# Cyan4973/FiniteStateEntropy

Measured on AMD Instinct MI355X. Metric: MB/s encode+decode per GPU on 32KB probagen blocks; bit-exact vs CPU ref, higher is better.
Workload: dtype u8; 1 GPU; probagen Proba14, 100000 x 32KB blocks per GPU, FSE encode+decode (one-shot calls at the reference's default limits: tableLog 11, decode maxLog 12), bit-exact check; blocks_per_gpu=100000, block_bytes=32768, codec=fse, parity=fse: roundtrip-all-blocks

## Files before the change

### finitestateentropy_amd/csrc/bitreader.h

```cpp
#pragma once
#include "dev_common.h"

enum { BR_UNFINISHED = 0, BR_END_OF_BUFFER = 1, BR_COMPLETED = 2, BR_OVERFLOW = 3 };

DEV u64 ldg64u(const u8* p) { u64 v; __builtin_memcpy(&v, p, 8); return v; }

struct BitReader {
    const u8* base; size_t size; size_t at; u64 win; u32 used;
    DEV size_t init(const u8* src, size_t n)
    {
        base = src; size = n; at = 0; win = 0; used = 0;
        if (n < 1) return FERR(srcSize_wrong);
        const u32 last = src[n - 1];
        if (n >= 8) {
            at = n - 8; win = ldg64u(src + at);
            if (last == 0) return FERR(GENERIC);
            used = 8 - hibit32(last);
        } else {
            for (size_t k = 0; k < n; ++k) win |= (u64)src[k] << (8 * k);
            if (last == 0) return FERR(corruption_detected);
            used = 8 - hibit32(last) + (u32)(8 - n) * 8;
        }
        return n;
    }
    DEV u32 read(u32 nb)
    {
        const u32 v = (u32)((win >> ((64u - used - nb) & 63u)) & (((u64)1 << nb) - 1));
        used += nb; return v;
    }
    DEV u32 read_fast(u32 nb)
    {
        const u32 v = (u32)((win << (used & 63u)) >> ((64u - nb) & 63u));
        used += nb; return v;
    }
    DEV int reload()
    {
        if (used > 64) return BR_OVERFLOW;
        if (at >= 8) { at -= used >> 3; used &= 7; win = ldg64u(base + at); return BR_UNFINISHED; }
        if (at == 0) return used < 64 ? BR_END_OF_BUFFER : BR_COMPLETED;
        u32 nbytes = used >> 3; int res = BR_UNFINISHED;
        if (at < nbytes) { nbytes = (u32)at; res = BR_END_OF_BUFFER; }
        at -= nbytes; used -= nbytes * 8; win = ldg64u(base + at);
        return res;
    }
};

DEV u32 fse_step(u32& state, BitReader& r, const u32* cells, bool fast)
{
    const u32 c = cells[state];
    const u32 nb = c >> 24;
    const u32 low = fast ? r.read_fast(nb) : r.read(nb);
    state = (c & 0xFFFFu) + low;
    return (c >> 16) & 0xFFu;
}
```

### finitestateentropy_amd/csrc/fse_decode.hip

```cpp
#include "internal.h"
#include <atomic>

#include "bitreader.h"

#ifndef FSE_SYM_L1
#define FSE_SYM_L1 1
#endif
#ifndef FSE_DEC_RING
#define FSE_DEC_RING 64
#endif
#define FSE_IN_RING 256
#define FSE_IN_RING_LOG 8
#define FSE_IN_CHUNK 64
#define FSE_IN_LANES (FSE_IN_CHUNK / 4)
#define FSE_IN_MIRROR 16
#ifndef FSE_CHECK_EVERY
#define FSE_CHECK_EVERY 16
#endif
#ifndef FSE_PHASE_UNROLL
#define FSE_PHASE_UNROLL 16
#endif
#define FSE_FINISH_EVERY 2
#ifndef FSE_DEC_LDS_KB
#define FSE_DEC_LDS_KB 160
// ... 133 lines not shown
DEV int ctl_peek(const int* p) { const int v = __hip_atomic_load(p, __ATOMIC_RELAXED, __HIP_MEMORY_SCOPE_WORKGROUP); __asm__ volatile("" ::: "memory"); return v; }
DEV void ctl_store(u32* p, u32 v) { __hip_atomic_store(p, v, __ATOMIC_RELEASE, __HIP_MEMORY_SCOPE_WORKGROUP); }
DEV u64 ctl_load2(const u32* p) { return __hip_atomic_load((const u64*)p, __ATOMIC_ACQUIRE, __HIP_MEMORY_SCOPE_WORKGROUP); }
DEV u64 ctl_peek2(const u32* p) { const u64 v = __hip_atomic_load((const u64*)p, __ATOMIC_RELAXED, __HIP_MEMORY_SCOPE_WORKGROUP); __asm__ volatile("" ::: "memory"); return v; }
DEV void ctl_store2(u32* p, u32 lo, u32 hi) { __hip_atomic_store((u64*)p, (u64)lo | ((u64)hi << 32), __ATOMIC_RELEASE, __HIP_MEMORY_SCOPE_WORKGROUP); }
DEV void ctl_store(int* p, int v) { __hip_atomic_store(p, v, __ATOMIC_RELEASE, __HIP_MEMORY_SCOPE_WORKGROUP); }

#define FSE_SRV_G 4
#ifndef FSE_FLUSH_MIN
#define FSE_FLUSH_MIN 32u
#endif
static_assert(FSE_SRV_WAVES * FSE_SRV_G == FSE_MAXG, "every block of a workgroup has a service wave");
static_assert((FSE_DEC_RING & (FSE_DEC_RING - 1)) == 0 && FSE_DEC_RING % FSE_CHECK_EVERY == 0, "ring positions wrap by masking; a phase never wraps");
DEV void fse_ring_put(u32* rg, int off, u32 w)
{
    const u32 j = (u32)off & (FSE_IN_RING - 1);
    rg[j >> 2] = w;
    if (j < FSE_IN_MIRROR) rg[(FSE_IN_RING + j) >> 2] = w;
}
DEV void fse_ring_put_rev(u32* rg, int Sg, int off, u32 w) { fse_ring_put(rg, ((Sg + 3) & ~3) - 4 - off, __brev(w)); }
DEV u32 fse_scratch_slot_claim(const FseDecArgs& a, u32* flagsSh)
{
    u32 slot = (u32)blockIdx.x % a.nSlots;
    for (;;) {
        const u32 bit = 1u << (slot & 31u);
        const u32 old = __hip_atomic_fetch_or(a.slotBitmap + (slot >> 5), bit, __ATOMIC_ACQUIRE, __HIP_MEMORY_SCOPE_AGENT);
        if (!(old & bit)) break;
        slot = slot + 1 == a.nSlots ? 0 : slot + 1;
    }
    flagsSh[6] = slot;
#if FSE_SYM_L1
    __builtin_amdgcn_fence(__ATOMIC_ACQUIRE, "agent");
#endif
    return slot;
}
DEV void fse_scratch_slot_done(const FseDecArgs& a, u32* flagsSh, int lane)
{
    if (lane == 0 && atomicAdd(&flagsSh[7], 1u) == FSE_SRV_WAVES + FSE_DEC_WAVES - 1) {
        const u32 slot = flagsSh[6];
        __hip_atomic_fetch_and(a.slotBitmap + (slot >> 5), ~(1u << (slot & 31u)), __ATOMIC_RELEASE, __HIP_MEMORY_SCOPE_AGENT);
    }
}
DEV u32 srv_rl(u32 v, int l) { return (u32)__builtin_amdgcn_readlane((int)v, l); }
DEV unsigned long long srv_rl64(unsigned long long v, int l) { return (unsigned long long)srv_rl((u32)v, l) | ((unsigned long long)srv_rl((u32)(v >> 32), l) << 32); }
template <bool TIMED, bool CALLER>
DEV void fse_decode_service(const FseDecArgs& a, u8* ldsb, DecCtl* ctlAll, u32 slotBytes, u32 ringOff, u32 inOff, int lane, int g0, bool rev, u32* flagsSh)
{
    const int myG = g0 + (lane < FSE_SRV_G ? lane : 0);
    DecCtl* const ctl = ctlAll + (myG < a.G ? myG : 0);
    const unsigned long long inBits = ((unsigned long long)ctl->inHi << 32) | ctl->inLo;
    const unsigned long long outBits = ((unsigned long long)ctl->outHi << 32) | ctl->outLo;
    const unsigned long long tabBits = ((unsigned long long)ctl->symHi << 32) | ctl->symLo;
    const int S32 = ctl->S32;
    int validLo = ctl->initValidLo;
    u32 flushed = 0, fpos = 0;
    bool live = lane < FSE_SRV_G && myG < a.G && !(ctl->pubPofs >> 31);

    static_assert(64 / FSE_IN_LANES == FSE_SRV_G, "one 16-lane group per block of a service wave");
    const int grp = lane / FSE_IN_LANES, sub = lane % FSE_IN_LANES;
    const int SgK = __shfl(S32, grp, WAVE);
    const gbl_u8_ptr igK = (gbl_u8_ptr)(uintptr_t)__shfl(inBits, grp, WAVE);
    u32* const rgK = (u32*)(ldsb + (size_t)(g0 + grp) * slotBytes + inOff);
    {   const bool liveK = (__ballot(live) >> grp) & 1ull;
        const int vlo = __shfl(validLo, grp, WAVE);
#pragma unroll
        for (int c = 0; c < FSE_IN_RING / FSE_IN_CHUNK; ++c) {
            const int off = liveK ? vlo + FSE_IN_CHUNK * c + 4 * sub : -1;
            if (off >= 0 && off + 4 <= SgK) { const u32 w = gbl_load_u32(igK + off); if (rev) fse_ring_put_rev(rgK, SgK, off, w); else fse_ring_put(rgK, off, w); }
            else if (off >= 0 && off < SgK) {
                u32 w = 0;
                for (int i = 0; i < 3; ++i) if (off + i < SgK) w |= (u32)igK[off + i] << (8 * i);
                if (rev) fse_ring_put_rev(rgK, SgK, off, w); else fse_ring_put(rgK, off, w);
            }
        }
        if (live) ctl_store(&ctl->srvValidLo, validLo);
    }

    int nextOff = __shfl(validLo, grp, WAVE) - FSE_IN_CHUNK + 4 * sub;
    u32 pend = 0;
    if (((__ballot(live) >> grp) & 1ull) && nextOff >= 0 && nextOff + 4 <= SgK) pend = gbl_load_u32(igK + nextOff);
    u32 yq[FSE_SRV_G][4];
#pragma unroll
    for (int l = 0; l < FSE_SRV_G; ++l) { yq[l][0] = yq[l][1] = yq[l][2] = yq[l][3] = 0; }
    unsigned long long sBusy = 0, sIdle = 0, nBusy = 0, sA = 0;
    (void)sBusy; (void)sIdle; (void)nBusy; (void)sA;
    TIMING(sA = __builtin_readcyclecounter(););
    for (;;) {
        u32 pp = 0x80000000u, it = flushed;
        if (live) { const u64 pub = ctl_load2(&ctl->pubIters); it = (u32)pub; pp = (u32)(pub >> 32); }
        const bool fin = (pp >> 31) != 0;
        const int P = (int)(pp & 0x7FFFFFFFu);
        const u32 avail = it - flushed;
        const bool wantFlush = live && (avail >= FSE_FLUSH_MIN || (fin && avail > 0));
        const bool wantFill = live && !fin && validLo > 0 && P + 4 <= validLo + (FSE_IN_RING - FSE_IN_CHUNK);
        const unsigned long long fm = __ballot(wantFlush), rm = __ballot(wantFill);
        if (live && fin && avail == 0) live = false;
        if (!(fm | rm)) {
            if (!__any(live)) break;
            __builtin_amdgcn_s_sleep(4);
            TIMING(const unsigned long long sB = __builtin_readcyclecounter(); sIdle += sB - sA; sA = sB;);
            continue;
        }
        const bool fillK = (rm >> grp) & 1ull;
        if (rm) {
            if (fillK) { if (rev) fse_ring_put_rev(rgK, SgK, nextOff, pend); else fse_ring_put(rgK, nextOff, pend); }
            if (wantFill) { validLo -= FSE_IN_CHUNK; ctl_store(&ctl->srvValidLo, validLo); }
            if (fillK) {
                nextOff -= FSE_IN_CHUNK;
                pend = 0;
                if (nextOff >= 0 && nextOff + 4 <= SgK) pend = gbl_load_u32(igK + nextOff);
            }
        }
#pragma unroll
        for (int l = 0; l < FSE_SRV_G; ++l) {
            if (!((fm >> l) & 1ull)) continue;
            const u32 cnt = srv_rl(avail, l), fp_g = srv_rl(fpos, l);
            const gbl_u8_ptr tg = (gbl_u8_ptr)(uintptr_t)srv_rl64(tabBits, l);
            if ((u32)lane < cnt) {
                u32 ri = fp_g + (u32)lane;
                ri = ri >= FSE_DEC_RING ? ri - FSE_DEC_RING : ri;
                const u32* const rw = (const u32*)(ldsb + (size_t)(g0 + l) * slotBytes + ringOff) + 4u * (ri >> 1) + (ri & 1u);
                uint2 rec; rec.x = rw[0]; rec.y = rw[2];
                const u32 x0 = __builtin_amdgcn_ubfe(rec.x, 1u, a.ldsLog), x1 = __builtin_amdgcn_ubfe(rec.x, 17u, a.ldsLog);
                const u32 x2 = __builtin_amdgcn_ubfe(rec.y, 1u, a.ldsLog), x3 = __builtin_amdgcn_ubfe(rec.y, 17u, a.ldsLog);
#if FSE_SYM_L1
                yq[l][0] = tg[x0]; yq[l][2] = tg[x1]; yq[l][1] = tg[x2]; yq[l][3] = tg[x3];
#else
                if (CALLER) {
                    yq[l][0] = __hip_atomic_load(tg + x0, __ATOMIC_RELAXED, __HIP_MEMORY_SCOPE_AGENT); yq[l][2] = __hip_atomic_load(tg + x1, __ATOMIC_RELAXED, __HIP_MEMORY_SCOPE_AGENT);
                    yq[l][1] = __hip_atomic_load(tg + x2, __ATOMIC_RELAXED, __HIP_MEMORY_SCOPE_AGENT); yq[l][3] = __hip_atomic_load(tg + x3, __ATOMIC_RELAXED, __HIP_MEMORY_SCOPE_AGENT);
                } else { yq[l][0] = tg[x0]; yq[l][2] = tg[x1]; yq[l][1] = tg[x2]; yq[l][3] = tg[x3]; }
#endif
            }
        }
        if (wantFlush) { ctl_store(&ctl->srvFlushed, it); }
#pragma unroll
        for (int l = 0; l < FSE_SRV_G; ++l) {
            if (!((fm >> l) & 1ull)) continue;
            const u32 cnt = srv_rl(avail, l), fl_g = srv_rl(flushed, l);
            gbl_u8_w_ptr const og = (gbl_u8_w_ptr)(uintptr_t)(srv_rl64(outBits, l) + 4ull * fl_g);
            if ((u32)lane < cnt) {
                const u32 w = yq[l][0] | (yq[l][1] << 8) | (yq[l][2] << 16) | (yq[l][3] << 24);
                gbl_store_u32(og + 4u * lane, w);
            }
        }
        if (wantFlush) { fpos += it - flushed; fpos = fpos >= FSE_DEC_RING ? fpos - FSE_DEC_RING : fpos; flushed = it; }
        TIMING(const unsigned long long sB = __builtin_readcyclecounter(); sBusy += sB - sA; sA = sB; ++nBusy;);
    }
    TIMING(if (lane == 0 && g0 == 0) { atomicAdd(&g_decTiming[5], sBusy); atomicAdd(&g_decTiming[6], sIdle); });
    if (CALLER) fse_scratch_slot_done(a, flagsSh, lane);
}

struct FseCellsRef { const u32* cells;
    DEV void get(u32 st, u32& ns, u32& nb, u32& sym) const { const u32 c = cells[st]; ns = c & 0xFFFFu; sym = (c >> 16) & 0xFFu; nb = c >> 24; } };
struct FseCellsCompact { const u16* A; const u8* syms;
    DEV void get(u32 st, u32& ns, u32& nb, u32& sym) const { const u32 c = A[st]; ns = c & 0xFFFu; nb = c >> 12; sym = syms[st]; } };
struct FseCellsRev { const u16* A; const u8* syms; u32 tl, cellShift;
    DEV void get(u32 st, u32& ns, u32& nb, u32& sym) const { const u32 i = __brev(st) >> (32u - tl); const u32 c = A[i]; nb = c & 31u; ns = __brev(c >> cellShift) >> (32u - tl); sym = syms[i]; } };
template <class Cells>
DEV u32 fse_tail_step(const Cells& t, u32& state, BitReader& r, bool fast)
{
    u32 ns, nb, sym;
    t.get(state, ns, nb, sym);
    const u32 low = fast ? r.read_fast(nb) : r.read(nb);
    state = ns + low;
    return sym;
}
template <class Cells>
DEV size_t fse_tail(const Cells& t, u32 s1, u32 s2, BitReader& r, u8* out, long op, long omax, bool fast)
{
    for (;;) {
        const int st = r.reload();
        if (!((st == BR_UNFINISHED) & (op < omax - 3))) break;
        u32 w = fse_tail_step(t, s1, r, fast);
        w |= fse_tail_step(t, s2, r, fast) << 8;
        w |= fse_tail_step(t, s1, r, fast) << 16;
        w |= fse_tail_step(t, s2, r, fast) << 24;
        __builtin_memcpy(out + op, &w, 4);
        op += 4;
    }
    for (;;) {
        if (op > omax - 2) return FERR(dstSize_tooSmall);
        out[op++] = (u8)fse_tail_step(t, s1, r, fast);
        if (r.reload() == BR_OVERFLOW) { out[op++] = (u8)fse_tail_step(t, s2, r, fast); return (size_t)op; }
        if (op > omax - 2) return FERR(dstSize_tooSmall);
        out[op++] = (u8)fse_tail_step(t, s2, r, fast);
        if (r.reload() == BR_OVERFLOW) { out[op++] = (u8)fse_tail_step(t, s1, r, fast); return (size_t)op; }
    }
}

template <bool FAST, bool TIMED, bool CALLER, bool VIEW = false>
__global__ __launch_bounds__(FSE_DEC_THREADS) void k_fse_decode(FseDecArgs a)
{
    extern __shared__ __attribute__((aligned(16))) u32 lds[];
    const int tid = threadIdx.x, lane = tid & 63, wave = tid >> 6;
    unsigned long long tBorn = 0, wBorn = 0;
    (void)tBorn; (void)wBorn;
    TIMING(tBorn = __builtin_readcyclecounter(); wBorn = wall_clock64(););
    const size_t first = (size_t)blockIdx.x * a.G;
    static_assert(FSE_DBINS % 4 == 0, "the bin lengths are read as 16-byte vectors");
    size_t nTot = a.nBlocks, q0 = first;
    u32 bin0 = 0, cnt0 = 0xFFFFFFFFu;
    if (a.count) {
        uint4 cv[FSE_DBINS / 4];
#pragma unroll
        for (u32 i = 0; i < FSE_DBINS / 4; ++i) cv[i] = ((const uint4*)a.count)[i];
        u64 before = 0;
        bool found = false;
#pragma unroll
        for (u32 i = 0; i < FSE_DBINS; ++i) {
            const uint4 v = cv[i >> 2];
            const u32 c = (i & 3u) == 0 ? v.x : (i & 3u) == 1 ? v.y : (i & 3u) == 2 ? v.z : v.w;
            const bool here = !found & (((u64)first < before + c) | (i == FSE_DBINS - 1));
            bin0 = here ? i : bin0; q0 = here ? (size_t)((u64)first - before) : q0; cnt0 = here ? c : cnt0;
            found |= here;
            before += c;
        }
        nTot = (size_t)before;
    }
    if (first >= nTot) return;
    auto slotBlock = [&](size_t g) -> size_t {
        if (!a.list) return first + g;
        size_t q = q0 + g; u32 i = bin0;
        if (q >= cnt0) {
            while (i < FSE_DBINS - 1) { const u32 c = a.count[i]; if (q < c) break; q -= c; ++i; }
        }
        return a.list[(size_t)i * a.nBlocks + q];
    };
    u8* const lds8 = (u8*)lds;
    const u32 tabStride = 2u << a.ldsLog;
    DecCtl* const ctlAll = (DecCtl*)(lds8 + (size_t)a.G * tabStride);
    u8* const ldsb = (u8*)ctlAll + (size_t)a.G * sizeof(DecCtl);
    const u32 slotBytes = a.slotU32 * 4u;
    const u32 ringOff = 0;
    const u32 inOff = FSE_DEC_RING * 8;

    u32* const flagsSh = (u32*)(ldsb + (size_t)a.G * slotBytes);
    if (tid < 6 || tid == 7) flagsSh[tid] = 0;
    const bool decWave = wave < FSE_DEC_WAVES;
    u8* const tlSh = (u8*)(flagsSh + 8);
    if (CALLER) {
        __syncthreads();
        bool mine = false;
        if (tid >= 64 && tid < 64 + a.G) {
            const size_t g = (size_t)tid - 64;
            u32 tl = 0xFFu;
            if (first + g < nTot) {
                const size_t bi = slotBlock(g);
                if (!(a.onlyDeclined && a.results[bi] != FSE_DECLINED)) {
                    const u32 t0 = a.dtables[bi * a.dtStrideU32] & 0xFFFFu;
                    if (t0 <= a.ldsLog && t0 >= a.tlMin) tl = t0;
                    else if (t0 > a.maxTableLog && a.tlMin == 0 && !a.onlyDeclined) a.results[bi] = FERR(tableLog_tooLarge);
                }
            }
            tlSh[g] = (u8)tl;
            mine = tl != 0xFFu;
        }
        if (mine) flagsSh[1] = 1u;
        u32 slot = 0;
        if (tid == 0) slot = fse_scratch_slot_claim(a, flagsSh);
        __syncthreads();
        if (!flagsSh[1]) {
            if (tid == 0) __hip_atomic_fetch_and(a.slotBitmap + (slot >> 5), ~(1u << (slot & 31u)), __ATOMIC_RELEASE, __HIP_MEMORY_SCOPE_AGENT);
            return;
        }
    }
    else __syncthreads();
    u8* const symSlot = CALLER ? a.symScratch + (size_t)flagsSh[6] * a.scratchSlotBytes : nullptr;
    {   u64 badBits = 0, declBits = 0; bool anyNb0 = false;
        if (!CALLER) {
            const size_t nTab = nTot - first < (size_t)a.G ? nTot - first : (size_t)a.G;
            if (tabStride >= 1024u) {
                const u32 ppt = tabStride >> 10;
                const u32 nPieces = (u32)nTab * ppt;
                for (u32 p = (u32)wave; p < nPieces; p += FSE_DEC_THREADS / 64) {
                    const u32 g = p / ppt, k = p - g * ppt;
                    const size_t bi = slotBlock(g);
                    const u8* const src = (const u8*)(a.atab + (bi << a.maxTableLog)) + 1024u * k + 16u * (u32)lane;
                    __builtin_amdgcn_global_load_lds((const __attribute__((address_space(1))) void*)src,
                                                     (__attribute__((address_space(3))) void*)(lds8 + 1024u * p), 16, 0, 0);
                }
            }
            else {
            uint4* const dstv = (uint4*)lds8;
            const u32 vptLog = a.ldsLog - 3u;
            const u32 nvec = (u32)nTab << vptLog;
            constexpr u32 MAXV = (FSE_MAXG * 512u / 16u + FSE_DEC_THREADS - 1) / FSE_DEC_THREADS;
            uint4 buf[MAXV];
#pragma unroll
            for (u32 k = 0; k < MAXV; ++k) {
                const u32 idx = tid + k * FSE_DEC_THREADS;
                if (idx < nvec) {
                    const size_t sl = first + (idx >> vptLog);
                    const size_t bi = slotBlock(sl - first);
                    buf[k] = ((const uint4*)(a.atab + (bi << a.maxTableLog)))[idx & ((1u << vptLog) - 1u)];
                }
            }
#pragma unroll
            for (u32 k = 0; k < MAXV; ++k) { const u32 idx = tid + k * FSE_DEC_THREADS; if (idx < nvec) dstv[idx] = buf[k]; }
            }
            if (!FAST) for (size_t g = 0; g < nTab; ++g) {
                const u32 st = a.meta[slotBlock(g)].state; anyNb0 |= st != 0 && !(st & 2u); }
        }
        else {
            const size_t nTab = nTot - first < (size_t)a.G ? nTot - first : (size_t)a.G;
            constexpr u32 QL = 2048u / 4u / 64u;
            if (!decWave) for (u32 g = (u32)wave - FSE_DEC_WAVES; g < (u32)nTab; g += FSE_SRV_WAVES) {
                const u32 tl = tlSh[g];
                if (tl == 0xFFu) continue;
                const u32 ts = 1u << tl;
                const u32* const t = a.dtables + slotBlock(g) * a.dtStrideU32;
                u8* const slotB = lds8 + (size_t)g * tabStride;
                u16* const A = (u16*)slotB;
                u8* const symOut = symSlot + ((size_t)g << a.ldsLog);
                bool bad = false, nbz = false;
                if (FAST && tl >= 4u) {
                    const u32 sR = 32u - tl;
                    const u32 qo[4] = { 0u, 1u << (tl - 1u), 1u << (tl - 2u), 3u << (tl - 2u) };
                    const u32 passes = ts > 2048u ? ts / 2048u : 1u;
                    u32 acc = 0, minNb = 15u;
                    uint4 cv[QL];
                    for (u32 h = 0; h < passes; ++h) {
#pragma unroll
                        for (u32 j = 0; j < QL; ++j) {
                            const u32 i0 = 2048u * h + 4u * ((u32)lane + 64u * j);
                            cv[j] = make_uint4(0, 0, 0, 0);
                            if (i0 < ts) __builtin_memcpy(&cv[j], t + 1 + i0, 16);
                        }
#pragma unroll
                        for (u32 j = 0; j < QL; ++j) {
                            const u32 i0 = 2048u * h + 4u * ((u32)lane + 64u * j);
                            if (i0 >= ts) continue;
                            const u32 r0 = __brev(i0) >> sR;
                            const u32 cw[4] = { cv[j].x, cv[j].y, cv[j].z, cv[j].w };
#pragma unroll
                            for (u32 q = 0; q < 4; ++q) {
                                const u32 c = cw[q], ns = c & 0xFFFFu, nb = c >> 24;
                                acc |= (ns >> tl) | ((tl - nb) >> 5) | (ns & ((1u << (nb & 31u)) - 1u));
                                minNb = nb < minNb ? nb : minNb;
                                slotB[r0 | qo[q]] = (u8)(c >> 16);
                            }
// ... 80 lines not shown
            s1 = r.read(tl); r.reload();
            s2 = r.read(tl); r.reload();
        }
    }

    __builtin_amdgcn_s_waitcnt(0x0f70);
    __syncthreads();
    const u64 badMask = (u64)flagsSh[2] | ((u64)flagsSh[3] << 32);
    const u64 declMask = (u64)flagsSh[4] | ((u64)flagsSh[5] << 32);
    const bool nb0 = flagsSh[0] != 0;
    if (CALLER && owner && a.declineNb0 && ((declMask >> gsl) & 1ull)) { if (half == 0) a.results[b] = FSE_DECLINED; owner = false; }

    const bool bulkOk = owner && S < (1ull << 28) && !((badMask >> gsl) & 1ull) && !(FAST && !compact && ((declMask >> gsl) & 1ull));
    const int Bstart = bulkOk ? (int)(8u * ((u32)r.at + 8u)) - (int)r.used : 0;
    const long groups0 = (omax - 3 - op + 3) / 4;
    bool can = bulkOk && (FAST ? Bstart >= 65 + 48 * (FSE_CHECK_EVERY - 1) : r.at >= 24 + 6 * FSE_CHECK_EVERY + 8) && groups0 >= FSE_CHECK_EVERY;
    bool can2 = FAST && bulkOk && Bstart >= 65 + 48 * (FSE_FINISH_EVERY - 1) && groups0 >= FSE_FINISH_EVERY;
    const bool everBulk = can || can2;
    BulkState bs; bs.q = 0; bs.bq = 0;
    {   const u32 st = half ? s2 : s1;
        bs.s = tabOff + 2u * (FAST ? __brev(st) >> (32u - (tl ? tl : 1u)) : st); }
    const u32 inA = (u32)((uintptr_t)in & 3u);
    const u32 R8 = 8u * (((u32)S + inA + 3u) & ~3u);
    u32 P = 0;
    long groups = 0;
    u32 iters = 0;
    int validLo = 0;
    if (everBulk) {
        const u32 B = 8u * ((u32)r.at + 8u + inA) - r.used;
        bs.q = 4u * (B >> 5) - 8u; bs.bq = B & 31u; P = R8 - B;
        groups = (omax - 3 - op + 3) >> 2;
        const int c0 = (int)((0 - ((uintptr_t)in - inA)) & (FSE_IN_CHUNK - 1));
        validLo = (((int)bs.q + 8 - 112 - c0) & ~(FSE_IN_CHUNK - 1)) + c0;
    }
    DecCtl* const ctl = ctlAll + (gsl < a.G ? gsl : 0);
    if (decWave && (lane >> 1) < ppw && gsl < a.G && half == 0) {
        ctl->pubIters = 0; ctl->pubPofs = everBulk ? bs.q + 8u : 0x80000000u;
        ctl->srvFlushed = 0; ctl->srvValidLo = 0x7FFFFFFF;
        ctl->initValidLo = validLo; ctl->S32 = (int)(S < (1ull << 31) ? S + inA : 0);
        const unsigned long long ib = (unsigned long long)(uintptr_t)(in - inA), ob = (unsigned long long)(uintptr_t)out, tb = (unsigned long long)(uintptr_t)syms;
        ctl->inLo = (u32)ib; ctl->inHi = (u32)(ib >> 32); ctl->outLo = (u32)ob; ctl->outHi = (u32)(ob >> 32); ctl->symLo = (u32)tb; ctl->symHi = (u32)(tb >> 32);
    }
    __syncthreads();
    if (!decWave) { fse_decode_service<TIMED, CALLER>(a, ldsb, ctlAll, slotBytes, ringOff, inOff, lane, (wave - FSE_DEC_WAVES) * FSE_SRV_G, FAST, flagsSh); return; }

    __builtin_amdgcn_s_setprio(3);
    uint2* const myRing = (uint2*)(ldsb + (size_t)(gsl < a.G ? gsl : 0) * slotBytes + ringOff) + half;
    const u32 myIn = (u32)(uintptr_t)(__attribute__((address_space(3))) u8*)(ldsb + (size_t)(gsl < a.G ? gsl : 0) * slotBytes + inOff);
    unsigned long long tRun = 0, tWait = 0, nRun = 0, nWait = 0, tA = 0, tFin = 0, nFin = 0, tInner = 0;
    (void)tRun; (void)tWait; (void)nRun; (void)nWait; (void)tA; (void)tFin; (void)nFin; (void)tInner;
    TIMING(tA = __builtin_readcyclecounter(););
    const unsigned long long tBulk0 = tA;
    (void)tBulk0;
    u32 rpos = 0;
    u64 srvNext = ctl_peek2(&ctl->srvFlushed);
    const u32 inA8 = 8u * inA;
    u32 Phead = P;
    int grp = groups > (1 << 30) ? (1 << 30) : (int)groups;
    if constexpr (FAST) {
        uint2* const dummyRing = (uint2*)(flagsSh + 32) + half;
        if ((lane >> 1) < ppw && everBulk) {
        for (;;) {
            const int lowest = (int)bs.q - 4 * ((48 * (FSE_CHECK_EVERY - 1) + 31) / 32);
            const int need = lowest > 0 ? lowest : 0;
            bool rdy;
            do {
                const u32 fl = (u32)srvNext;
                const int vlo = (int)(u32)(srvNext >> 32);
                srvNext = ctl_peek2(&ctl->srvFlushed);
                rdy = !can | ((iters + FSE_CHECK_EVERY - fl <= FSE_DEC_RING) & (need >= vlo));
                TIMING(if (!__all(rdy)) { const unsigned long long tB = __builtin_readcyclecounter(); tWait += tB - tA; ++nWait; tA = tB; });
            } while (!__all(rdy));
            if (!__any(can)) break;
            uint2* const ring = can ? myRing + rpos : dummyRing;
            u32 sN = bs.s, Pn = P, PhN = Phead;
            unsigned long long tI = 0; (void)tI;
            TIMING(tI = __builtin_readcyclecounter(););
            fse_bulk_phase_rev<FSE_CHECK_EVERY>(sN, Pn, PhN, tl + 1u, 4u, tabOff, myIn, maskB & 31u, ring);
            TIMING(tInner += __builtin_readcyclecounter() - tI;);
            bs.s = can ? sN : bs.s; P = can ? Pn : P; Phead = can ? PhN : Phead;
            const u32 adv = can ? (u32)FSE_CHECK_EVERY : 0u;
            rpos = (rpos + adv) & (FSE_DEC_RING - 1);
            iters += adv; grp -= (int)adv;
            const u32 B = R8 - P;
            bs.q = 4u * (B >> 5) - 8u;
            const u32 Bp = B - inA8;
            const bool canN = can & (Bp >= 65u + 48u * (FSE_CHECK_EVERY - 1)) & (grp >= FSE_CHECK_EVERY);
            const bool more = canN | ((Bp >= 65u + 48u * (FSE_FINISH_EVERY - 1)) & (grp >= FSE_FINISH_EVERY));
            if (can & (half == 0)) ctl_store2(&ctl->pubIters, iters, more ? bs.q + 8u : ((bs.q + 8u) | 0x80000000u));
            can = canN;
            TIMING(const unsigned long long tB = __builtin_readcyclecounter(); tRun += tB - tA; ++nRun; tA = tB;);
        }
        {   const u32 B = R8 - P; bs.bq = B & 31u;
            can2 = bulkOk & (B - inA8 >= 65u + 48u * (FSE_FINISH_EVERY - 1)) & (grp >= FSE_FINISH_EVERY); }
        can2 = can2 & bulkOk;
        for (;;) {
            const u32 fl = (u32)srvNext;
            const int vlo = (int)(u32)(srvNext >> 32);
            srvNext = ctl_peek2(&ctl->srvFlushed);
            const int lowest = (int)bs.q - 8;
            const bool rdy = !can2 | ((iters + FSE_FINISH_EVERY - fl <= FSE_DEC_RING) & ((lowest > 0 ? lowest : 0) >= vlo));
            if (!__all(rdy)) {
                TIMING(const unsigned long long tB = __builtin_readcyclecounter(); tWait += tB - tA; ++nWait; tA = tB;);
                continue;
            }
            if (!__any(can2)) break;
            uint2* const ring = can2 ? myRing + rpos : dummyRing;
            u32 sN = bs.s, Pn = P, PhN = Phead;
            fse_bulk_phase_rev<FSE_FINISH_EVERY>(sN, Pn, PhN, tl + 1u, 4u, tabOff, myIn, maskB & 31u, ring);
            bs.s = can2 ? sN : bs.s; P = can2 ? Pn : P; Phead = can2 ? PhN : Phead;
            rpos = can2 ? (rpos + FSE_FINISH_EVERY) & (FSE_DEC_RING - 1) : rpos;
            iters += can2 ? FSE_FINISH_EVERY : 0u; grp -= can2 ? FSE_FINISH_EVERY : 0;
            const u32 B = R8 - P;
            bs.q = 4u * (B >> 5) - 8u; bs.bq = B & 31u;
            const bool can2N = can2 & (B - inA8 >= 65u + 48u * (FSE_FINISH_EVERY - 1)) & (grp >= FSE_FINISH_EVERY);
            if (can2 & (half == 0)) ctl_store2(&ctl->pubIters, iters, can2N ? bs.q + 8u : ((bs.q + 8u) | 0x80000000u));
            can2 = can2N;
            TIMING(const unsigned long long tB = __builtin_readcyclecounter(); tFin += tB - tA; ++nFin; tA = tB;);
        }
        }
    } else {
    while (__any(can)) {
        const u32 fl = (u32)srvNext;
        const int vlo = (int)(u32)(srvNext >> 32);
        srvNext = ctl_peek2(&ctl->srvFlushed);
        const int lowest = (int)bs.q - (6 * FSE_CHECK_EVERY + 8);
        const bool ready = can & (iters + FSE_CHECK_EVERY - fl <= FSE_DEC_RING) & ((lowest > 0 ? lowest : 0) >= vlo);
        if (ready) {
            uint2* const ring = myRing + rpos;
            rpos = (rpos + FSE_CHECK_EVERY) & (FSE_DEC_RING - 1);
            if (nb0) fse_bulk_phase<true>(bs.s, bs.q, bs.bq, tabOff, myIn, half, maskB, ring);
            else     fse_bulk_phase<false>(bs.s, bs.q, bs.bq, tabOff, myIn, half, maskB, ring);
            iters += FSE_CHECK_EVERY; grp -= FSE_CHECK_EVERY;
            can = (bs.q >= 24u + 6u * FSE_CHECK_EVERY + 4u) & (grp >= FSE_CHECK_EVERY);
            if (half == 0) ctl_store2(&ctl->pubIters, iters, can ? bs.q + 8u : ((bs.q + 8u) | 0x80000000u));
        }
        TIMING(const unsigned long long tB = __builtin_readcyclecounter(); if (__any(ready)) { tRun += tB - tA; ++nRun; } else { tWait += tB - tA; ++nWait; } tA = tB;);
    }
    }
    TIMING(if (lane == 0) { atomicAdd(&g_decTiming[0], tRun); atomicAdd(&g_decTiming[1], tWait); atomicAdd(&g_decTiming[2], nRun); atomicAdd(&g_decTiming[3], nWait); atomicAdd(&g_decTiming[4], 1ull);
                            atomicAdd(&g_decTiming[13], tBulk0 - tBorn); atomicAdd(&g_decTiming[15], tFin); atomicAdd(&g_decTiming[10], nFin); atomicAdd(&g_decTiming[7], tInner); });
    const u32 sOther = dpp_swap(bs.s);
    const unsigned long long tBulk1 = tA;
    (void)tBulk1;
    if (owner && !half) {
    op = 4 * (long)iters;
    if (iters) {
        const u32 B = 8u * (bs.q + 8u) + bs.bq - 8u * inA;
        const u32 Bh = FAST ? R8 - Phead - 8u * inA : B;
        r.at = (size_t)((Bh + 7u) >> 3) - 8; r.used = 8u * ((u32)r.at + 8u) - B; r.win = ldg64u(in + r.at); s1 = (bs.s - tabOff) >> 1; s2 = (sOther - tabOff) >> 1;
        if (FAST) { s1 = __brev(s1) >> (32u - tl); s2 = __brev(s2) >> (32u - tl); }
    }

    size_t result;
    if (!compact) {
        if ((badMask >> gsl) & 1ull) result = fse_tail(FseCellsRef{cells}, s1, s2, r, out, op, omax, fast);
        else if (FAST)               result = fse_tail(FseCellsRev{A, syms, tl, 5u}, s1, s2, r, out, op, omax, fast);
        else                         result = fse_tail(FseCellsCompact{A, syms}, s1, s2, r, out, op, omax, fast);
    }
    else if (FAST)    result = fse_tail(FseCellsRev{A, syms, tl, 5u}, s1, s2, r, out, op, omax, fast);
    else              result = fse_tail(FseCellsCompact{A, syms}, s1, s2, r, out, op, omax, fast);
    a.results[b] = result;
    TIMING(if (lane == 0) { const unsigned long long tE = __builtin_readcyclecounter(); atomicAdd(&g_decTiming[11], tE - tBorn); atomicAdd(&g_decTiming[12], wall_clock64() - wBorn);
                            atomicAdd(&g_decTiming[14], tE - tBulk1); });
    }
    if (CALLER) fse_scratch_slot_done(a, flagsSh, lane);
}

static void fse_decode_geometry(unsigned ldsLog, size_t ldsBytes, unsigned* slotU32, int* G)
{
    *slotU32 = (FSE_DEC_RING * 8 + FSE_IN_RING + FSE_IN_MIRROR + 16) / 4;
    int g = (int)((ldsBytes - 256) / ((2u << ldsLog) + *slotU32 * 4 + sizeof(DecCtl)));
    if (g > FSE_MAXG) g = FSE_MAXG;
    *G = g;
}
#define FSE_DEC_LDS (FSE_DEC_LDS_KB * 1024)
size_t fse_decode_blocks_per_round(unsigned maxTableLog)
{
    unsigned slot; int G;
    fse_decode_geometry(maxTableLog < FSE_DEC_FAST_MAXLOG ? maxTableLog : FSE_DEC_FAST_MAXLOG, FSE_DEC_LDS, &slot, &G);
    const int cus = dev_props().ok ? dev_props().cus : 256;
    return (size_t)G * FSE_WGS_PER_CU * cus;
}

#define FSE_SYM_SLOT_BYTES (FSE_MAXG * 2048u)
#include <mutex>
namespace {
std::mutex g_symMutex;
struct SymScratch { u8* base = nullptr; u32* bitmap = nullptr; u32 nSlots = 0; };
SymScratch g_symScratch[64];
}
static hipError_t fse_sym_scratch(FseDecArgs& a, hipStream_t s)
{
    int dev = 0;
    hipError_t e = hipGetDevice(&dev);
    if (e != hipSuccess) return e;
    if (dev < 0 || dev >= 64) return hipErrorInvalidDevice;
    std::lock_guard<std::mutex> lock(g_symMutex);
    SymScratch& sc = g_symScratch[dev];
    if (!sc.base && s) {
        hipStreamCaptureStatus st = hipStreamCaptureStatusNone;
        if (hipStreamIsCapturing(s, &st) == hipSuccess && st != hipStreamCaptureStatusNone) return hipErrorStreamCaptureUnsupported;
        (void)hipGetLastError();
    }
    if (!sc.base) {
        const u32 nSlots = 2u * (u32)(dev_props().ok ? dev_props().cus : 256);
        const size_t bitmapBytes = ((nSlots + 31u) / 32u * 4u + 255u) & ~(size_t)255;
        u8* p = nullptr;
        e = hipMalloc((void**)&p, bitmapBytes + (size_t)nSlots * FSE_SYM_SLOT_BYTES);
        if (e != hipSuccess) return e;
        e = hipMemset(p, 0, bitmapBytes);
        if (e != hipSuccess) { (void)hipFree(p); return e; }
        sc.bitmap = (u32*)p; sc.base = p + bitmapBytes; sc.nSlots = nSlots;
    }
    a.symScratch = sc.base; a.slotBitmap = sc.bitmap; a.nSlots = sc.nSlots; a.scratchSlotBytes = FSE_SYM_SLOT_BYTES;
    return hipSuccess;
}

static hipError_t fse_decode_launch(FseDecArgs a, bool rev, hipStream_t s)
{
    const size_t ldsBytes = FSE_DEC_LDS;
    const bool caller = a.atab == nullptr;
    {   hipError_t e = ensure_dyn_lds((const void*)k_fse_decode<true, false, false>, FSE_DEC_LDS);
        if (e == hipSuccess) e = ensure_dyn_lds((const void*)k_fse_decode<false, false, false>, FSE_DEC_LDS);
        if (e == hipSuccess) e = ensure_dyn_lds((const void*)k_fse_decode<true, true, false>, FSE_DEC_LDS);
        if (e == hipSuccess && caller) e = ensure_dyn_lds((const void*)k_fse_decode<true, false, true>, FSE_DEC_LDS);
        if (e == hipSuccess && caller) e = ensure_dyn_lds((const void*)k_fse_decode<false, false, true>, FSE_DEC_LDS);
        if (e == hipSuccess && caller) e = fse_sym_scratch(a, s);
        if (e != hipSuccess) return e;
    }
    fse_decode_geometry(a.ldsLog, ldsBytes, &a.slotU32, &a.G);
    if (a.G < 1) return hipErrorInvalidValue;
    if (caller && ((size_t)a.G << a.ldsLog) > FSE_SYM_SLOT_BYTES) return hipErrorInvalidValue;
    const size_t groups = (a.nBlocks + a.G - 1) / a.G;
    if (a.dstOffsets) {
        if (caller || !a.dstCaps) return hipErrorInvalidValue;
        hipError_t e = ensure_dyn_lds((const void*)k_fse_decode<true, false, false, true>, FSE_DEC_LDS);
        if (e == hipSuccess) e = ensure_dyn_lds((const void*)k_fse_decode<false, false, false, true>, FSE_DEC_LDS);
        if (e != hipSuccess) return e;
        if (rev) hipLaunchKernelGGL((k_fse_decode<true, false, false, true>), dim3((unsigned)groups), dim3(FSE_DEC_THREADS), ldsBytes, s, a);
        else     hipLaunchKernelGGL((k_fse_decode<false, false, false, true>), dim3((unsigned)groups), dim3(FSE_DEC_THREADS), ldsBytes, s, a);
        return hipGetLastError();
    }
    if (caller) {
        if (rev && g_decTimingOn.load(std::memory_order_relaxed)) {
            hipError_t e = ensure_dyn_lds((const void*)k_fse_decode<true, true, true>, FSE_DEC_LDS);
            if (e != hipSuccess) return e;
            hipLaunchKernelGGL((k_fse_decode<true, true, true>), dim3((unsigned)groups), dim3(FSE_DEC_THREADS), ldsBytes, s, a);
        }
        else if (rev) hipLaunchKernelGGL((k_fse_decode<true, false, true>), dim3((unsigned)groups), dim3(FSE_DEC_THREADS), ldsBytes, s, a);
        else     hipLaunchKernelGGL((k_fse_decode<false, false, true>), dim3((unsigned)groups), dim3(FSE_DEC_THREADS), ldsBytes, s, a);
    }
    else if (rev && g_decTimingOn.load(std::memory_order_relaxed)) hipLaunchKernelGGL((k_fse_decode<true, true, false>), dim3((unsigned)groups), dim3(FSE_DEC_THREADS), ldsBytes, s, a);
    else if (rev) hipLaunchKernelGGL((k_fse_decode<true, false, false>), dim3((unsigned)groups), dim3(FSE_DEC_THREADS), ldsBytes, s, a);
    else          hipLaunchKernelGGL((k_fse_decode<false, false, false>), dim3((unsigned)groups), dim3(FSE_DEC_THREADS), ldsBytes, s, a);
    return hipGetLastError();
}

extern "C" __attribute__((visibility("default"))) int FSEHIP_prepareDevice(void)
{
    FseDecArgs a = FseDecArgs();
    return (int)fse_sym_scratch(a, nullptr);
}

extern "C" __attribute__((visibility("default"))) int FSEHIP_debug_decodeTiming(int enable, unsigned long long* out16)
{
    hipError_t e = hipDeviceSynchronize();
    if (e != hipSuccess) return (int)e;
    if (enable) {
        unsigned long long zero[16] = { 0 };
        e = hipMemcpyToSymbol(HIP_SYMBOL(g_decTiming), zero, sizeof(zero));
        g_decTimingOn.store(e == hipSuccess);
        return (int)e;
    }
    g_decTimingOn.store(false);
    if (!out16) return 0;
    e = hipMemcpyFromSymbol(out16, HIP_SYMBOL(g_decTiming), sizeof(g_decTiming));
    if (e != hipSuccess) return (int)e;
    int dev = 0, khz = 0;
    (void)hipGetDevice(&dev);
    (void)hipDeviceGetAttribute(&khz, hipDeviceAttributeClockRate, dev);
    unsigned slot; int G;
    fse_decode_geometry(FSE_DEC_FAST_MAXLOG, FSE_DEC_LDS, &slot, &G);
    out16[8] = (unsigned long long)khz; out16[9] = (unsigned long long)G | ((unsigned long long)FSE_WGS_PER_CU << 32) | ((unsigned long long)FSE_DEC_WAVES << 40) | ((unsigned long long)FSE_CHECK_EVERY << 48);
    return 0;
}

hipError_t launch_fse_decode(FseDecArgs a, hipStream_t s)
{
    if (a.nBlocks == 0) return hipSuccess;
    a.list = nullptr; a.count = nullptr;
    probe_before(PK_FSE_DECODE, s);
    a.ldsLog = a.maxTableLog < FSE_DEC_FAST_MAXLOG ? a.maxTableLog : FSE_DEC_FAST_MAXLOG;
    a.tlMin = 0; a.declineNb0 = 0; a.onlyDeclined = 0;
    hipError_t e = fse_decode_launch(a, true, s);
    if (e == hipSuccess && a.maxTableLog > FSE_DEC_FAST_MAXLOG) {
        a.ldsLog = a.maxTableLog; a.tlMin = FSE_DEC_FAST_MAXLOG + 1; a.declineNb0 = 1;
        e = fse_decode_launch(a, true, s);
        if (e == hipSuccess) { a.tlMin = 0; a.declineNb0 = 0; a.onlyDeclined = 1; e = fse_decode_launch(a, false, s); }
    }
    probe_after(PK_FSE_DECODE, s);
    return e;
}

hipError_t launch_fse_decode_classes(FseDecArgs a, const u32* lists, const u32* counts, hipStream_t s)
{
    if (a.nBlocks == 0) return hipSuccess;
    probe_before(PK_FSE_DECODE, s);
    hipError_t e = hipSuccess;
    for (int c = 0; c < FSE_DCLS_KINDS && e == hipSuccess; ++c) {
        if (c != FSE_DCLS_REV11 && a.maxTableLog <= FSE_DEC_FAST_MAXLOG) break;
        a.list = lists + (size_t)c * FSE_DBINS * a.nBlocks; a.count = counts + c * FSE_DBINS;
        a.ldsLog = c == FSE_DCLS_REV11 ? (a.maxTableLog < FSE_DEC_FAST_MAXLOG ? a.maxTableLog : FSE_DEC_FAST_MAXLOG) : a.maxTableLog;
        e = fse_decode_launch(a, c != FSE_DCLS_PLAIN, s);
// ... 5 lines not shown
```

Measured before the change: 207,300 MiB/s of uncompressed data through encode+decode (whole job).

## Cache final bitstream bytes in registers and defer symbol lookups in decode tail

Adds a windowed bit reader that, once the read position nears the stream start, captures the last 16-24 bytes into registers so later reloads avoid dependent global loads. The tail decoder is restructured to first run the state chain for a bounded number of quads and singles, saving table indices (tokens), then resolve symbols and write output afterward. This takes the symbol-table load off the serial state-update chain. In exchange it adds register pressure and more complex code in the per-block tail, which only affects the end of each block.

```diff
diff --git a/finitestateentropy_amd/csrc/bitreader.h b/finitestateentropy_amd/csrc/bitreader.h
--- a/finitestateentropy_amd/csrc/bitreader.h
+++ b/finitestateentropy_amd/csrc/bitreader.h
@@ -1,5 +1,7 @@
 #pragma once
+#ifndef BITREADER_HOST
 #include "dev_common.h"
+#endif
 
 enum { BR_UNFINISHED = 0, BR_END_OF_BUFFER = 1, BR_COMPLETED = 2, BR_OVERFLOW = 3 };
 
@@ -45,6 +47,63 @@
     }
 };
 
+struct WinBitReader {
+    const u8* base; size_t size; size_t at; u64 win; u32 used;
+    u64 w0, w1, w2; bool reg;
+    DEV void from(const BitReader& r)
+    {
+        base = r.base; size = r.size; at = r.at; used = r.used;
+        w0 = w1 = w2 = 0; reg = false;
+        settle(r.win);
+    }
+    DEV u64 window(u32 p) const
+    {
+        const u32 k = p >> 3, sh = 8u * (p & 7u);
+        const u64 x0 = w0, x1 = w1, x2 = w2;
+        const u64 a = k == 0 ? x0 : k == 1 ? x1 : x2, b = k == 0 ? x1 : k == 1 ? x2 : 0;
+        return sh ? (a >> sh) | (b << (64u - sh)) : a;
+    }
+    DEV void settle(u64 nw)
+    {
+        const bool cap = !reg & (at <= 16);
+        u64 n0 = w0, n1 = w1, n2 = w2;
+        if (cap) {
+            const u32 p = (u32)at;
+            u64 lo = 0, mid = 0;
+            if (size >= 8) { lo = ldg64u(base); mid = ldg64u(base + (p < 8u ? p : 8u)); }
+            const u64 below = nw >> ((8u * (8u - p)) & 63u), above = nw >> ((8u * (16u - p)) & 63u);
+            n0 = lo; n1 = p >= 8u ? mid : p ? below : 0; n2 = p > 8u ? above : 0;
+        }
+        const bool nreg = reg | cap;
+        win = nw; w0 = n0; w1 = n1; w2 = n2; reg = nreg;
+    }
+    DEV void load()
+    {
+        u64 nw;
+        if (reg) nw = window((u32)at); else nw = ldg64u(base + at);
+        settle(nw);
+    }
+    DEV u32 read(u32 nb)
+    {
+        const u32 v = (u32)((win >> ((64u - used - nb) & 63u)) & (((u64)1 << nb) - 1));
+        used += nb; return v;
+    }
+    DEV u32 read_fast(u32 nb)
+    {
+        const u32 v = (u32)((win << (used & 63u)) >> ((64u - nb) & 63u));
+        used += nb; return v;
+    }
+    DEV int reload()
+    {
+        if (used > 64) return BR_OVERFLOW;
+        if (at == 0) return used < 64 ? BR_END_OF_BUFFER : BR_COMPLETED;
+        u32 nbytes = used >> 3; int res = BR_UNFINISHED;
+        if (at < nbytes) { nbytes = (u32)at; res = BR_END_OF_BUFFER; }
+        at -= nbytes; used -= nbytes * 8; load();
+        return res;
+    }
+};
+
 DEV u32 fse_step(u32& state, BitReader& r, const u32* cells, bool fast)
 {
     const u32 c = cells[state];
diff --git a/finitestateentropy_amd/csrc/fse_decode.hip b/finitestateentropy_amd/csrc/fse_decode.hip
--- a/finitestateentropy_amd/csrc/fse_decode.hip
+++ b/finitestateentropy_amd/csrc/fse_decode.hip
@@ -309,41 +309,126 @@
 }
 
 struct FseCellsRef { const u32* cells;
-    DEV void get(u32 st, u32& ns, u32& nb, u32& sym) const { const u32 c = cells[st]; ns = c & 0xFFFFu; sym = (c >> 16) & 0xFFu; nb = c >> 24; } };
+    DEV void get(u32 st, u32& ns, u32& nb, u32& tok) const { const u32 c = cells[st]; ns = c & 0xFFFFu; tok = (c >> 16) & 0xFFu; nb = c >> 24; }
+    DEV u32 sym(u32 tok) const { return tok; } };
 struct FseCellsCompact { const u16* A; const u8* syms;
-    DEV void get(u32 st, u32& ns, u32& nb, u32& sym) const { const u32 c = A[st]; ns = c & 0xFFFu; nb = c >> 12; sym = syms[st]; } };
+    DEV void get(u32 st, u32& ns, u32& nb, u32& tok) const { const u32 c = A[st]; ns = c & 0xFFFu; nb = c >> 12; tok = st; }
+    DEV u32 sym(u32 tok) const { return syms[tok]; } };
 struct FseCellsRev { const u16* A; const u8* syms; u32 tl, cellShift;
-    DEV void get(u32 st, u32& ns, u32& nb, u32& sym) const { const u32 i = __brev(st) >> (32u - tl); const u32 c = A[i]; nb = c & 31u; ns = __brev(c >> cellShift) >> (32u - tl); sym = syms[i]; } };
-template <class Cells>
-DEV u32 fse_tail_step(const Cells& t, u32& state, BitReader& r, bool fast)
-{
-    u32 ns, nb, sym;
-    t.get(state, ns, nb, sym);
+    DEV void get(u32 st, u32& ns, u32& nb, u32& tok) const { const u32 i = __brev(st) >> (32u - tl); const u32 c = A[i]; nb = c & 31u; ns = __brev(c >> cellShift) >> (32u - tl); tok = i; }
+    DEV u32 sym(u32 tok) const { return syms[tok]; } };
+template <class Cells, class Reader>
+DEV u32 fse_tail_step(const Cells& t, u32& state, Reader& r, bool fast)
+{
+    u32 ns, nb, tok;
+    t.get(state, ns, nb, tok);
     const u32 low = fast ? r.read_fast(nb) : r.read(nb);
     state = ns + low;
-    return sym;
-}
-template <class Cells>
-DEV size_t fse_tail(const Cells& t, u32 s1, u32 s2, BitReader& r, u8* out, long op, long omax, bool fast)
+    return tok;
+}
+template <class Cells, class Reader>
+DEV void fse_tail_quads(const Cells& t, u32& s1, u32& s2, Reader& r, u8* out, long& op, long omax, bool fast)
 {
     for (;;) {
         const int st = r.reload();
         if (!((st == BR_UNFINISHED) & (op < omax - 3))) break;
-        u32 w = fse_tail_step(t, s1, r, fast);
-        w |= fse_tail_step(t, s2, r, fast) << 8;
-        w |= fse_tail_step(t, s1, r, fast) << 16;
-        w |= fse_tail_step(t, s2, r, fast) << 24;
+        u32 w = t.sym(fse_tail_step(t, s1, r, fast));
+        w |= t.sym(fse_tail_step(t, s2, r, fast)) << 8;
+        w |= t.sym(fse_tail_step(t, s1, r, fast)) << 16;
+        w |= t.sym(fse_tail_step(t, s2, r, fast)) << 24;
         __builtin_memcpy(out + op, &w, 4);
         op += 4;
     }
+}
+template <class Cells, class Reader>
+DEV size_t fse_tail_singles(const Cells& t, u32 s1, u32 s2, Reader& r, u8* out, long op, long omax, bool fast)
+{
     for (;;) {
         if (op > omax - 2) return FERR(dstSize_tooSmall);
-        out[op++] = (u8)fse_tail_step(t, s1, r, fast);
-        if (r.reload() == BR_OVERFLOW) { out[op++] = (u8)fse_tail_step(t, s2, r, fast); return (size_t)op; }
+        out[op++] = (u8)t.sym(fse_tail_step(t, s1, r, fast));
+        if (r.reload() == BR_OVERFLOW) { out[op++] = (u8)t.sym(fse_tail_step(t, s2, r, fast)); return (size_t)op; }
         if (op > omax - 2) return FERR(dstSize_tooSmall);
-        out[op++] = (u8)fse_tail_step(t, s2, r, fast);
-        if (r.reload() == BR_OVERFLOW) { out[op++] = (u8)fse_tail_step(t, s1, r, fast); return (size_t)op; }
-    }
+        out[op++] = (u8)t.sym(fse_tail_step(t, s2, r, fast));
+        if (r.reload() == BR_OVERFLOW) { out[op++] = (u8)t.sym(fse_tail_step(t, s1, r, fast)); return (size_t)op; }
+    }
+}
+template <int N>
+struct FseTokQuads {
+    u64 q[N];
+    DEV void clear() {
+#pragma unroll
+        for (int j = 0; j < N; ++j) q[j] = 0; }
+    DEV void push(u64 w) {
+#pragma unroll
+        for (int j = N - 1; j > 0; --j) q[j] = q[j - 1];
+        q[0] = w; }
+};
+#ifndef FSE_TAIL_QUADS
+#define FSE_TAIL_QUADS 6
+#endif
+#ifndef FSE_TAIL_SINGLES
+#define FSE_TAIL_SINGLES 6
+#endif
+template <class Cells, class Reader>
+DEV size_t fse_tail(const Cells& t, u32 s1, u32 s2, Reader& r, u8* out, long op, long omax, bool fast)
+{
+    FseTokQuads<FSE_TAIL_QUADS> qa; qa.clear();
+    const long opA = op;
+    u32 nA = 0;
+    bool ended = false;
+    while (nA < FSE_TAIL_QUADS) {
+        const int st = r.reload();
+        if (!((st == BR_UNFINISHED) & (op < omax - 3))) { ended = true; break; }
+        u64 w = (u64)(fse_tail_step(t, s1, r, fast) & 0xFFFFu);
+        w |= (u64)(fse_tail_step(t, s2, r, fast) & 0xFFFFu) << 16;
+        w |= (u64)(fse_tail_step(t, s1, r, fast) & 0xFFFFu) << 32;
+        w |= (u64)(fse_tail_step(t, s2, r, fast) & 0xFFFFu) << 48;
+        qa.push(w); ++nA; op += 4;
+    }
+    u32 ya[FSE_TAIL_QUADS][4];
+#pragma unroll
+    for (int j = 0; j < FSE_TAIL_QUADS; ++j)
+#pragma unroll
+        for (int k = 0; k < 4; ++k) ya[j][k] = t.sym((u32)(qa.q[j] >> (16 * k)) & 0xFFFFu);
+    FseTokQuads<FSE_TAIL_SINGLES> qb; qb.clear();
+    const long opB = op;
+    u32 nB = 0;
+    u64 cur = 0;
+    size_t result = 0;
+    bool done = false;
+    auto single = [&](u32& s) { cur |= (u64)(fse_tail_step(t, s, r, fast) & 0xFFFFu) << (16u * (nB & 3u)); ++nB; ++op; if (!(nB & 3u)) { qb.push(cur); cur = 0; } };
+    if (ended) while (nB + 3u <= 4u * FSE_TAIL_SINGLES) {
+        if (op > omax - 2) { result = FERR(dstSize_tooSmall); done = true; break; }
+        single(s1);
+        if (r.reload() == BR_OVERFLOW) { single(s2); result = (size_t)op; done = true; break; }
+        if (op > omax - 2) { result = FERR(dstSize_tooSmall); done = true; break; }
+        single(s2);
+        if (r.reload() == BR_OVERFLOW) { single(s1); result = (size_t)op; done = true; break; }
+    }
+    if (nB & 3u) qb.push(cur);
+    const u32 gB = (nB + 3u) >> 2;
+    u32 yb[FSE_TAIL_SINGLES][4];
+#pragma unroll
+    for (int j = 0; j < FSE_TAIL_SINGLES; ++j)
+#pragma unroll
+        for (int k = 0; k < 4; ++k) yb[j][k] = t.sym((u32)(qb.q[j] >> (16 * k)) & 0xFFFFu);
+#pragma unroll
+    for (int j = 0; j < FSE_TAIL_QUADS; ++j) if ((u32)j < nA) {
+        const u32 w = ya[j][0] | (ya[j][1] << 8) | (ya[j][2] << 16) | (ya[j][3] << 24);
+        __builtin_memcpy(out + opA + 4 * (long)(nA - 1u - (u32)j), &w, 4);
+    }
+#pragma unroll
+    for (int j = 0; j < FSE_TAIL_SINGLES; ++j) if ((u32)j < gB) {
+        const u32 g = gB - 1u - (u32)j, left = nB - 4u * g;
+        u8* const o = out + opB + 4 * (long)g;
+        o[0] = (u8)yb[j][0];
+        if (left > 1u) o[1] = (u8)yb[j][1];
+        if (left > 2u) o[2] = (u8)yb[j][2];
+        if (left > 3u) o[3] = (u8)yb[j][3];
+    }
+    if (done) return result;
+    if (!ended) fse_tail_quads(t, s1, s2, r, out, op, omax, fast);
+    return fse_tail_singles(t, s1, s2, r, out, op, omax, fast);
 }
 
 template <bool FAST, bool TIMED, bool CALLER, bool VIEW = false>
@@ -730,14 +815,15 @@
         if (FAST) { s1 = __brev(s1) >> (32u - tl); s2 = __brev(s2) >> (32u - tl); }
     }
 
+    WinBitReader wr; wr.from(r);
     size_t result;
     if (!compact) {
-        if ((badMask >> gsl) & 1ull) result = fse_tail(FseCellsRef{cells}, s1, s2, r, out, op, omax, fast);
-        else if (FAST)               result = fse_tail(FseCellsRev{A, syms, tl, 5u}, s1, s2, r, out, op, omax, fast);
-        else                         result = fse_tail(FseCellsCompact{A, syms}, s1, s2, r, out, op, omax, fast);
-    }
-    else if (FAST)    result = fse_tail(FseCellsRev{A, syms, tl, 5u}, s1, s2, r, out, op, omax, fast);
-    else              result = fse_tail(FseCellsCompact{A, syms}, s1, s2, r, out, op, omax, fast);
+        if ((badMask >> gsl) & 1ull) result = fse_tail(FseCellsRef{cells}, s1, s2, wr, out, op, omax, fast);
+        else if (FAST)               result = fse_tail(FseCellsRev{A, syms, tl, 5u}, s1, s2, wr, out, op, omax, fast);
+        else                         result = fse_tail(FseCellsCompact{A, syms}, s1, s2, wr, out, op, omax, fast);
+    }
+    else if (FAST)    result = fse_tail(FseCellsRev{A, syms, tl, 5u}, s1, s2, wr, out, op, omax, fast);
+    else              result = fse_tail(FseCellsCompact{A, syms}, s1, s2, wr, out, op, omax, fast);
     a.results[b] = result;
     TIMING(if (lane == 0) { const unsigned long long tE = __builtin_readcyclecounter(); atomicAdd(&g_decTiming[11], tE - tBorn); atomicAdd(&g_decTiming[12], wall_clock64() - wBorn);
                             atomicAdd(&g_decTiming[14], tE - tBulk1); });
```

Measured after the change: 207,700 MiB/s of uncompressed data through encode+decode (whole job) (median of 6 runs). Within noise of the previous version (+0.2%).
